# kwea123/nsff_pl

Hardware: AMD Instinct MI355X
Metric: ray-samples/sec (coarse+fine, static+dynamic) (higher is better)
Workload: dtype f16x3 (fp32 operands split into 2 halfs, 3 f16 MFMAs per product, fp32 accumulate; same 1e-4 parity as f32); 1 GPU; C2 (BASELINE.json configs[1]): static+dynamic NSFF, 1024 rays/GPU x (64 coarse + 64 importance -> 192 fine pts), train-mode fwd, fw/bw flow warp t+-1, perturb=1 noise_std=1, 8x256 MLPs, N_tau=48, all 47 outputs on device.  `value` is render_rays' throughput with autograd DISABLED (the train-mode FLAGS, inference launches: nothing kept for a backward pass); what a trainer's forward costs is aux.tra; rays_per_gpu=1024, N_samples=64, N_importance=64, parallelism=single GPU, field_launch=persistent (one workgroup per CU)

## Files before the change

### include/nsff_render.h

```cpp
#ifndef NSFF_RENDER_H
#define NSFF_RENDER_H

#include <stddef.h>
#include <stdint.h>

#ifdef __cplusplus
extern "C" {
#endif

#define NSFF_OK               0
#define NSFF_ERR_INVALID     -1
#define NSFF_ERR_NULL        -2
#define NSFF_ERR_ALIGN       -3
#define NSFF_ERR_HIP         -4

#define NSFF_ABI_VERSION      32
#define NSFF_RAW_STRIDE      16
#define NSFF_MAX_FREQS       24
#define NSFF_MAX_LAYERS       8


typedef struct NsffModelDesc {
    int32_t D;
    int32_t W;
// ... 275 lines not shown
    const float* xyz_bw;
    const float* noise_static;
    const float* noise_transient;
    const float* noise_fw;
    const float* noise_bw;
    const float* visibility;
    float* static_rgbs;  float* transient_rgbs;
    float* flows_fw;     float* flows_bw;
    float* static_sigmas; float* transient_sigmas;
    float* static_alphas; float* transient_alphas;
    float* static_weights; float* transient_weights; float* weights;
    float* xyzs_fw_bw;   float* xyzs_bw_fw;
    float* disoccs_fw;   float* disoccs_bw;
    float* depth;  float* rgb;  float* transient_alpha;  float* transient_rgb;
    float* static_only_rgb;  float* static_only_depth;
    float* xyz_exp;  float* flow_fw_exp;  float* flow_bw_exp;  float* xyz_fw_exp;  float* xyz_bw_exp;
    float* rgb_fw;   float* rgb_bw;
    float* disocc_fw;  float* disocc_bw;
    NsffFrustumArgs vis;
} NsffCompositeArgs;

int nsff_composite(const NsffCompositeArgs* args, void* stream);

int nsff_frustum_visibility(const NsffFrustumArgs* vis, const float* xyz, int64_t n_points, float* vis_count,
                            void* stream);

typedef struct NsffSplatArgs {
    int32_t H, W, n_planes;
    float   K4[4];
    float   P[12];
    float   scale;
    const float* xyz;
    const float* flow;
    const float* rgb;
    const float* alpha;
    float*       accum;
    void*        work;
    int64_t      work_bytes;
} NsffSplatArgs;
int64_t nsff_splat_work_bytes(int32_t H, int32_t W, int32_t n_planes);
int nsff_splat_planes(const NsffSplatArgs* args, void* stream);

typedef struct NsffMpiArgs {
    int32_t H, W, n_planes;
    float   dt;
    const float* accum_fw;
// ... 104 lines not shown
```

### nsff_pl_amd/_lib.py

```python
import ctypes as C
import os

import torch

_HERE = os.path.dirname(os.path.abspath(__file__))
LIB_PATH = os.environ.get("NSFF_LIB") or os.path.join(_HERE, "libnsff_hip.so")

RAW_STRIDE = 16
ABI_VERSION = 32
MAX_FREQS = 24

_ERR = {-1: "NSFF_ERR_INVALID (bad shape/flag/unsupported architecture)",
        -2: "NSFF_ERR_NULL (required pointer missing)",
        -3: "NSFF_ERR_ALIGN (pointer not 16-byte aligned)",
        -4: "NSFF_ERR_HIP"}

_fp = C.c_void_p


class ModelDesc(C.Structure):
    _fields_ = [("D", C.c_int32), ("W", C.c_int32), ("skip", C.c_int32),
                ("in_xyz", C.c_int32), ("in_dir", C.c_int32), ("in_a", C.c_int32),
                ("in_t", C.c_int32), ("use_viewdir", C.c_int32),
                ("has_transient", C.c_int32), ("has_flow", C.c_int32),
# ... 153 lines not shown
    "nsff_field_launch_plan": (C.c_int, [C.POINTER(ModelDesc), C.POINTER(FieldArgs), C.c_int32, C.c_int32, C.POINTER(C.c_int32), C.c_int32]),
    "nsff_time_bias_rows": (C.c_int, [C.POINTER(ModelDesc)]),
    "nsff_time_bias": (C.c_int, [C.POINTER(TimeBiasJob), C.c_int32, C.c_int64, C.c_void_p]),
    "nsff_rng_draws": (C.c_int, [C.POINTER(RngJob), C.c_int32, C.c_uint64, C.c_void_p]),
    "nsff_rng_draws_coarse": (C.c_int, [C.POINTER(RngJob), C.c_int32, C.c_uint64, C.POINTER(RngCoarse), C.c_void_p]),
    "nsff_side_bias": (C.c_int, [C.POINTER(ModelDesc), _fp, _fp, _fp, _fp, C.c_int64, _fp, C.c_void_p]),
    "nsff_last_hip_error": (C.c_char_p, []),
    "nsff_packed_bytes": (C.c_int, [C.POINTER(ModelDesc), C.c_int, C.POINTER(C.c_size_t)]),
    "nsff_param_count": (C.c_int, [C.POINTER(ModelDesc)]),
    "nsff_pack_weights": (C.c_int, [C.POINTER(ModelDesc), C.c_int, C.POINTER(_fp), _fp, _fp]),
    "nsff_pack_weights_ex": (C.c_int, [C.POINTER(ModelDesc), C.c_int, C.POINTER(_fp), _fp, C.c_int32, _fp]),
    "nsff_fold_heads": (C.c_int, [C.POINTER(ModelDesc), C.c_int, C.POINTER(_fp), _fp, _fp]),
    "nsff_posenc": (C.c_int, [_fp, C.c_int64, C.POINTER(C.c_float), C.c_int, _fp, _fp]),
    "nsff_time_rows": (C.c_int, [_fp, C.c_int64, C.c_int32, _fp, C.c_int64, C.c_int64, _fp, _fp, _fp]),
    "nsff_time_rows_backward": (C.c_int, [_fp, _fp, _fp, _fp, C.c_int64, C.c_int64, C.c_int64, C.c_int32, _fp, _fp]),
    "nsff_field_query": (C.c_int, [C.POINTER(ModelDesc), _fp, C.POINTER(FieldArgs), _fp]),
    "nsff_coarse_samples": (C.c_int, [_fp, C.c_int64, _fp, C.c_int32, C.c_float, _fp, _fp, _fp, _fp]),
    "nsff_fine_samples": (C.c_int, [_fp, C.c_int64, _fp, _fp, C.c_int32, C.c_int32, _fp, _fp, _fp, _fp,
                                    C.c_int32, _fp, _fp, _fp, _fp, _fp]),
    "nsff_sample_pdf": (C.c_int, [_fp, _fp, C.c_int64, C.c_int32, _fp, C.c_int32, C.c_int32,
                                  C.c_float, _fp, _fp]),
    "nsff_warp_points": (C.c_int, [_fp, _fp, _fp, C.c_int64, C.c_float, _fp, _fp, _fp]),
    "nsff_composite": (C.c_int, [C.POINTER(CompositeArgs), _fp]),
    "nsff_frustum_visibility": (C.c_int, [C.POINTER(FrustumArgs), _fp, C.c_int64, _fp, _fp]),
    "nsff_frame_rays": (C.c_int, [C.POINTER(C.c_float), C.POINTER(C.c_float), C.c_int32, C.c_int32, C.c_float,
                                  C.c_float, C.c_int64, C.c_int64, _fp, _fp]),
    "nsff_bwd_packed_bytes": (C.c_int, [C.POINTER(ModelDesc), C.POINTER(C.c_size_t)]),
    "nsff_pack_weights_bwd": (C.c_int, [C.POINTER(ModelDesc), C.POINTER(_fp), _fp, _fp]),
    "nsff_field_backward": (C.c_int, [C.POINTER(ModelDesc), _fp, C.POINTER(FieldBwdArgs), _fp]),
    "nsff_field_input_backward": (C.c_int, [_fp, C.c_int32, C.c_int32, _fp, C.c_int64, C.c_int32, C.POINTER(C.c_float), C.c_int32,
                                            C.c_int32, _fp, _fp, _fp]),
    "nsff_train_dims": (C.c_int, [C.POINTER(ModelDesc), C.POINTER(C.c_int32), C.POINTER(C.c_int32), C.POINTER(C.c_int32)]),
    "nsff_weight_grad_scratch": (C.c_int64, [C.POINTER(WgradJob), C.c_int32, C.c_int64, C.c_int32]),
    "nsff_weight_grad": (C.c_int, [C.POINTER(WgradJob), C.c_int32, C.c_int64, C.c_int32, _fp, _fp, _fp, _fp, _fp]),
    "nsff_weight_grad_accumulate": (C.c_int, [C.POINTER(WgradJob), C.c_int32, C.c_int64, C.c_int32, _fp, _fp, C.c_int64,
                                              _fp, _fp, _fp]),
    "nsff_weight_grad_accumulate_aux": (C.c_int, [C.POINTER(WgradJob), C.c_int32, C.c_int64, C.c_int32, _fp, _fp, C.c_int64,
                                                  _fp, _fp, _fp, _fp]),
    "nsff_absmax_raw": (C.c_int, [_fp, C.c_int64, _fp, _fp]),
    "nsff_last_bwd_kernel": (C.c_int, []),
    "nsff_last_bwd_grid": (C.c_int, []),
    "nsff_field_bwd_phase_program": (C.c_int, [C.POINTER(ModelDesc), C.c_int32, C.c_int32, C.c_int64, C.POINTER(C.c_uint32), C.c_int32,
                                                C.POINTER(C.c_uint32), C.c_int32]),
    "nsff_field_bwd_launch_plan": (C.c_int, [C.POINTER(ModelDesc), C.POINTER(FieldBwdArgs), C.c_int32, C.c_int32, C.c_int32,
                                             C.POINTER(C.c_int32), C.c_int32]),
    "nsff_fold_grads": (C.c_int, [C.POINTER(FoldGradArgs), _fp]),
# ... 399 lines not shown
                                  _ptr(u), samples.shape[1], int(u_per_ray), float(eps),
                                  _ptr(samples), _stream()), "nsff_sample_pdf")


def warp_points(raw, xyz, zs, z_far, xyz_fw, xyz_bw):
    _check(load().nsff_warp_points(_ptr(raw), _ptr(xyz), _ptr(zs), zs.numel(), float(z_far),
                                   _ptr(xyz_fw), _ptr(xyz_bw), _stream()), "nsff_warp_points")


def frustum_args(w2c, ts, K4, n_cams, n_frames, H, W):
    assert w2c.is_cuda and w2c.dtype == torch.float32 and w2c.is_contiguous() and w2c.shape == (n_cams * n_frames, 12)
    assert ts.is_cuda and ts.dtype == torch.int64 and ts.is_contiguous() and ts.numel() >= 1
    a = FrustumArgs(w2c=w2c.data_ptr(), ts=ts.data_ptr(), n_cams=int(n_cams), n_frames=int(n_frames), H=int(H), W=int(W))
    a.K4[:] = [float(v) for v in K4]
    a._keep = (w2c, ts)
    return a


def frustum_visibility(vis, xyz, out):
    _check(load().nsff_frustum_visibility(C.byref(vis), _ptr(xyz), xyz.shape[0], _ptr(out), _stream()),
           "nsff_frustum_visibility")


def composite(vis=None, **kw):
    a = CompositeArgs()
    for k, v in kw.items():
        if k in _COMPOSITE_PTRS_IN or k in _COMPOSITE_PTRS_OUT:
            setattr(a, k, _ptr(v))
        else:
            setattr(a, k, v)
    if vis is not None:
        a.vis = vis
    _check(load().nsff_composite(C.byref(a), _stream()), "nsff_composite")


def frame_rays(K4, c2w12, H, W, near, shift_near, first, count, rays):
    k = (C.c_float * 4)(*[float(v) for v in K4])
    m = (C.c_float * 12)(*[float(v) for v in c2w12])
    _check(load().nsff_frame_rays(k, m, int(H), int(W), float(near), float(shift_near), int(first), int(count),
                                  _ptr(rays), _stream()), "nsff_frame_rays")


BWD_PACK = 100


def bwd_packed_bytes(desc):
    n = C.c_size_t(0)
    _check(load().nsff_bwd_packed_bytes(C.byref(desc), C.byref(n)), "nsff_bwd_packed_bytes")
    return n.value


def pack_weights_bwd(desc, params, packed, fwd_packed=None):
    arr = (_fp * len(params))(*[p.data_ptr() for p in params])
    _check(load().nsff_pack_weights_bwd_ex(C.byref(desc), arr, _ptr(packed), _ptr(fwd_packed), _stream()), "nsff_pack_weights_bwd_ex")


# ... 300 lines not shown
```

### nsff_pl_amd/csrc/rays.hip

```cpp
#include <hip/hip_runtime.h>
#include <cstdlib>
#include "nsff_common.h"

namespace {

constexpr int WAVES_PER_BLOCK = 4;
constexpr int RS = NSFF_RAW_STRIDE;

__device__ __forceinline__ float wave_sum(float v) {
#pragma unroll
    for (int off = 32; off > 0; off >>= 1) v += __shfl_xor(v, off);
    return v;
}

__device__ __forceinline__ float wave_scan_mul(float v, int lane) {
#pragma unroll
    for (int off = 1; off < 64; off <<= 1) {
        const float u = __shfl_up(v, off);
        if (lane >= off) v *= u;
    }
    return v;
}
__device__ __forceinline__ float wave_scan_add(float v, int lane) {
#pragma unroll
// ... 52 lines not shown
        const int below = max(lo - 1, 0), above = min(lo, M);
        const float cb = cdf[below], ca = cdf[above];
        const float bb = bins[below], ba = bins[above];
        float denom = ca - cb;
        if (denom < eps) denom = 1.f;
        const float s = bb + (uk - cb) / denom * (ba - bb);
        if (active) {
            if (out_a) out_a[k] = s;
            if (out_b) out_b[k] = s;
        }
    }
    __syncthreads();
}

struct FineArgs {
    const float* rays; long long n_rays; const float* z_lin; const float* zs_coarse;
    int S, n_imp;
    const float* w_static; const float* w_transient;
    const float* u_static; const float* u_transient; int u_per_ray;
    float* samples_static; float* samples_transient;
    float* zs_fine; float* xyz_fine;
};

__global__ __launch_bounds__(64 * WAVES_PER_BLOCK) void fine_samples_kernel(const FineArgs a) {
    extern __shared__ __attribute__((aligned(16))) float smem[];
    const int lane = threadIdx.x & 63, wave = threadIdx.x >> 6, tid = threadIdx.x;
    constexpr int T = 64 * WAVES_PER_BLOCK;
    const long long ray = blockIdx.x;
    const int S = a.S, n_imp = a.n_imp;
    const int k_sets = a.w_transient ? 2 : 1;
    const int Sf = S + k_sets * n_imp;
    float* cdf = smem + wave * S;
    float* bins = smem + WAVES_PER_BLOCK * S;
    float* merged = bins + ((S + 3) & ~3);
    for (int j = tid; j < S - 1; j += T) bins[j] = 0.5f * (a.z_lin[j] + a.z_lin[j + 1]);
    for (int j = tid; j < S; j += T) merged[j] = a.zs_coarse[ray * S + j];
    __syncthreads();
    {
        const bool mine = wave < k_sets;
        const int set = mine ? wave : 0;
        const float* w = (set == 0 ? a.w_static : a.w_transient) + ray * S + 1;
        const float* ub = set == 0 ? a.u_static : a.u_transient;
        const float* u = a.u_per_ray ? ub + ray * n_imp : ub;
        float* keep = set == 0 ? a.samples_static : a.samples_transient;
        sample_pdf_ray(w, bins, S - 2, 1e-5f, u, n_imp, cdf, merged + S + set * n_imp,
                       keep ? keep + ray * n_imp : nullptr, lane, mine);
    }
    const float* r = a.rays + ray * 6;
    const float o0 = r[0], o1 = r[1], o2 = r[2], d0 = r[3], d1 = r[4], d2 = r[5];
    for (int i = tid; i < Sf; i += T) {
        const float v = merged[i];
        int rank = 0;
        int j = 0;
        for (; j + 4 <= Sf; j += 4) {
            const float4 o = *reinterpret_cast<const float4*>(merged + j);
            rank += (o.x < v || (o.x == v && j < i)) ? 1 : 0;
            rank += (o.y < v || (o.y == v && j + 1 < i)) ? 1 : 0;
            rank += (o.z < v || (o.z == v && j + 2 < i)) ? 1 : 0;
            rank += (o.w < v || (o.w == v && j + 3 < i)) ? 1 : 0;
        }
        for (; j < Sf; ++j) {
            const float o = merged[j];
            rank += (o < v || (o == v && j < i)) ? 1 : 0;
        }
        const long long dst = ray * Sf + rank;
        a.zs_fine[dst] = v;
        a.xyz_fine[dst * 3 + 0] = o0 + d0 * v;
        a.xyz_fine[dst * 3 + 1] = o1 + d1 * v;
        a.xyz_fine[dst * 3 + 2] = o2 + d2 * v;
    }
}

struct PdfArgs {
    const float* bins; const float* weights; long long n_rays; int M;
    const float* u; int n_imp; int u_per_ray; float eps; float* samples;
};

__global__ __launch_bounds__(64 * WAVES_PER_BLOCK) void sample_pdf_kernel(const PdfArgs a) {
    extern __shared__ __attribute__((aligned(16))) float smem[];
    const int lane = threadIdx.x & 63, wave = threadIdx.x >> 6;
    const long long ray_raw = (long long)blockIdx.x * WAVES_PER_BLOCK + wave;
    const bool active = ray_raw < a.n_rays;
    const long long ray = active ? ray_raw : a.n_rays - 1;
    float* cdf = smem + wave * (a.M + 1);
    const float* u = a.u_per_ray ? a.u + ray * a.n_imp : a.u;
    sample_pdf_ray(a.weights + ray * a.M, a.bins + ray * (a.M + 1), a.M, a.eps, u, a.n_imp, cdf,
                   active ? a.samples + ray * a.n_imp : nullptr, nullptr, lane, true);
}

struct FrameRayArgs {
    float fx, fy, cx, cy;
    float c2w[12];
    int W;
// ... 50 lines not shown
    const float ry = -rz * y * cy / fy;
    const long long frame = v.ts[0];
    float count = 0.f;
    if (frame < 0 || frame >= v.n_frames) return count;
    for (int c = 0; c < v.n_cams; ++c) {
        const float* m = v.w2c + ((long long)c * v.n_frames + frame) * 12;
        const float cam0 = fmaf(m[2], rz, fmaf(m[1], ry, m[0] * rx)) + m[3];
        const float cam1 = fmaf(m[6], rz, fmaf(m[5], ry, m[4] * rx)) + m[7];
        const float cam2 = fmaf(m[10], rz, fmaf(m[9], ry, m[8] * rx)) + m[11];
        if (!(cam2 < 0.f)) continue;
        const float c1 = -cam1, c2 = -cam2;
        const float u = fmaf(cx, c2, fx * cam0) / c2, w = fmaf(cy, c2, fy * c1) / c2;
        if (u >= 0.f && u < (float)v.W && w >= 0.f && w < (float)v.H) count += 1.f;
    }
    return count;
}

__global__ __launch_bounds__(256) void frustum_visibility_kernel(const NsffFrustumArgs v, const float* __restrict__ xyz,
                                                                 long long n_points, float* __restrict__ out) {
    const long long p = (long long)blockIdx.x * 256 + threadIdx.x;
    if (p < n_points) out[p] = frustum_count(v, xyz[3 * p], xyz[3 * p + 1], xyz[3 * p + 2]);
}

__global__ __launch_bounds__(64 * WAVES_PER_BLOCK) void composite_kernel(const NsffCompositeArgs a) {
    const int lane = threadIdx.x & 63;
    const long long ray = (long long)blockIdx.x * WAVES_PER_BLOCK + (threadIdx.x >> 6);
    if (ray >= a.n_rays) return;
    const int S = a.n_samples;
    const bool tr = a.has_transient != 0;
    const bool flows = tr && a.flow_mode >= 1;
    const bool warps = tr && a.flow_mode >= 2;

    float cT = 1.f, cTs = 1.f, cTfw = 1.f, cTbw = 1.f;
    float s_depth = 0.f, s_rgb[3] = {0, 0, 0}, s_talpha = 0.f, s_trgb[3] = {0, 0, 0};
    float s_sorgb[3] = {0, 0, 0}, s_sodepth = 0.f;
    float s_xyz[3] = {0, 0, 0}, s_ffw[3] = {0, 0, 0}, s_fbw[3] = {0, 0, 0};
    float s_rgbfw[3] = {0, 0, 0}, s_rgbbw[3] = {0, 0, 0}, s_occfw = 0.f, s_occbw = 0.f;

    for (int base = 0; base < S; base += 64) {
        const int i = base + lane;
        const bool on = i < S;
        const long long idx = ray * S + (on ? i : S - 1);
        const float z = a.zs[idx];
        const bool last = i >= S - 1;
        const float dz = last ? 0.f : a.zs[idx + 1] - z;
        const float d_s = last ? 100.f : dz;
        const float d_t = last ? 1e-3f : dz;
        const float* rec = a.raw + idx * RS;

        float sig_s = rec[3];
// ... 23 lines not shown
        cT *= __shfl(inc, 63);
        const float w = alpha * T, w_s = al_s * T, w_t = al_t * T;

        if (on) {
            if (a.static_sigmas) a.static_sigmas[idx] = sig_s;
            if (a.has_rgb && a.static_rgbs) {
                a.static_rgbs[idx * 3 + 0] = rgb_s[0]; a.static_rgbs[idx * 3 + 1] = rgb_s[1];
                a.static_rgbs[idx * 3 + 2] = rgb_s[2];
            }
            if (tr) {
                if (a.transient_sigmas) a.transient_sigmas[idx] = sig_t;
                if (a.has_rgb && a.transient_rgbs) {
                    a.transient_rgbs[idx * 3 + 0] = rgb_t[0]; a.transient_rgbs[idx * 3 + 1] = rgb_t[1];
                    a.transient_rgbs[idx * 3 + 2] = rgb_t[2];
                }
                if (a.static_alphas) a.static_alphas[idx] = al_s;
                if (a.transient_alphas) a.transient_alphas[idx] = al_t;
                if (a.static_weights) a.static_weights[idx] = w_s;
                if (a.transient_weights) a.transient_weights[idx] = w_t;
                if (a.weights) a.weights[idx] = w;
            } else {
                if (a.static_weights) a.static_weights[idx] = w;
                if (a.weights) a.weights[idx] = w;
            }
        }
        if (!a.has_rgb) continue;

        if (on) {
            s_depth += w * z;
            if (tr) {
#pragma unroll
                for (int c = 0; c < 3; ++c) { s_rgb[c] += w_s * rgb_s[c]; s_trgb[c] += w_t * rgb_t[c]; }
                s_talpha += w_t;
            } else {
#pragma unroll
                for (int c = 0; c < 3; ++c) s_rgb[c] += w * rgb_s[c];
            }
        }
        if (!tr) continue;

        {
            const float oms = on ? 1.f - al_s : 1.f;
            const float incs = wave_scan_mul(oms, lane);
            float excs = __shfl_up(incs, 1);
            if (lane == 0) excs = 1.f;
            const float Ts = cTs * excs;
// ... 89 lines not shown
        if (a.static_only_rgb) a.static_only_rgb[ray * 3 + c] = s_sorgb[c];
    }
    if (a.transient_alpha) a.transient_alpha[ray] = s_talpha;
    if (a.static_only_depth) a.static_only_depth[ray] = s_sodepth;
    if (flows) {
        for (int c = 0; c < 3; ++c) {
            if (a.xyz_exp) a.xyz_exp[ray * 3 + c] = s_xyz[c];
            if (a.flow_fw_exp) a.flow_fw_exp[ray * 3 + c] = s_ffw[c];
            if (a.flow_bw_exp) a.flow_bw_exp[ray * 3 + c] = s_fbw[c];
            if (a.xyz_fw_exp) a.xyz_fw_exp[ray * 3 + c] = s_xyz[c] + s_ffw[c];
            if (a.xyz_bw_exp) a.xyz_bw_exp[ray * 3 + c] = s_xyz[c] + s_fbw[c];
        }
    }
    if (warps) {
        for (int c = 0; c < 3; ++c) {
            if (a.rgb_fw) a.rgb_fw[ray * 3 + c] = s_rgbfw[c];
            if (a.rgb_bw) a.rgb_bw[ray * 3 + c] = s_rgbbw[c];
        }
        if (a.disocc_fw) a.disocc_fw[ray] = 1.f - fabsf(s_occfw);
        if (a.disocc_bw) a.disocc_bw[ray] = 1.f - fabsf(s_occbw);
    }
}

template <int NCH>
__global__ __launch_bounds__(64 * NCH) void composite_kernel_chunks(const NsffCompositeArgs a) {
    __shared__ float tot[NCH][4];
    __shared__ float part[NCH][32];
    const int lane = threadIdx.x & 63, c = threadIdx.x >> 6;
    const long long ray = blockIdx.x;
    const int S = a.n_samples;
    const bool tr = a.has_transient != 0;
    const bool flows = tr && a.flow_mode >= 1;
    const bool warps = tr && a.flow_mode >= 2;

    const int i = 64 * c + lane;
    const bool on = i < S;
    const long long idx = ray * S + (on ? i : S - 1);
    const float z = a.zs[idx];
    const bool last = i >= S - 1;
    const float dz = last ? 0.f : a.zs[idx + 1] - z;
    const float d_s = last ? 100.f : dz;
    const float d_t = last ? 1e-3f : dz;
    const float* rec = a.raw + idx * RS;

    float sig_s = rec[3];
    if (a.noise_static) sig_s += a.noise_static[idx] * a.noise_std;
    sig_s = softplus(sig_s);
    const float al_s = 1.f - expf(-d_s * sig_s);
    float rgb_s[3] = {0, 0, 0};
    if (a.has_rgb) { rgb_s[0] = rec[0]; rgb_s[1] = rec[1]; rgb_s[2] = rec[2]; }

    float sig_t = 0.f, al_t = 0.f, alpha = al_s;
    float rgb_t[3] = {0, 0, 0};
    if (tr) {
        sig_t = rec[7];
        if (a.visibility && a.visibility[idx] == 0.f) sig_t = -10.f;
        if (a.vis.w2c && frustum_count(a.vis, a.xyz[idx * 3], a.xyz[idx * 3 + 1], a.xyz[idx * 3 + 2]) == 0.f) sig_t = -10.f;
        if (a.noise_transient) sig_t += a.noise_transient[idx] * a.noise_std;
        sig_t = softplus(sig_t);
        al_t = 1.f - expf(-d_t * sig_t);
        alpha = 1.f - (1.f - al_s) * (1.f - al_t);
        if (a.has_rgb) { rgb_t[0] = rec[4]; rgb_t[1] = rec[5]; rgb_t[2] = rec[6]; }
    }
    const float inc = wave_scan_mul(on ? 1.f - alpha : 1.f, lane);
    float incs = 1.f, incw[2] = {1.f, 1.f}, al_tw[2] = {0.f, 0.f};
    if (a.has_rgb && tr) incs = wave_scan_mul(on ? 1.f - al_s : 1.f, lane);
    if (a.has_rgb && warps) {
#pragma unroll
        for (int dir = 0; dir < 2; ++dir) {
            const float* recw = (dir == 0 ? a.raw_fw : a.raw_bw) + idx * RS;
            const float* nz = dir == 0 ? a.noise_fw : a.noise_bw;
            float sg = recw[7];
            if (nz) sg += nz[idx] * a.noise_std;
            al_tw[dir] = 1.f - expf(-d_t * softplus(sg));
            const float al_w = 1.f - (1.f - al_s) * (1.f - al_tw[dir]);
            incw[dir] = wave_scan_mul(on ? 1.f - al_w : 1.f, lane);
        }
    }
    if (lane == 63) { tot[c][0] = inc; tot[c][1] = incs; tot[c][2] = incw[0]; tot[c][3] = incw[1]; }
    __syncthreads();
    float cT = 1.f, cTs = 1.f, cTw[2] = {1.f, 1.f};
    for (int cc = 0; cc < c; ++cc) { cT *= tot[cc][0]; cTs *= tot[cc][1]; cTw[0] *= tot[cc][2]; cTw[1] *= tot[cc][3]; }

    float exc = __shfl_up(inc, 1);
    if (lane == 0) exc = 1.f;
    const float T = cT * exc;
    const float w = alpha * T, w_s = al_s * T, w_t = al_t * T;
    if (on) {
        if (a.static_sigmas) a.static_sigmas[idx] = sig_s;
        if (a.has_rgb && a.static_rgbs) {
            a.static_rgbs[idx * 3 + 0] = rgb_s[0]; a.static_rgbs[idx * 3 + 1] = rgb_s[1];
            a.static_rgbs[idx * 3 + 2] = rgb_s[2];
        }
        if (tr) {
            if (a.transient_sigmas) a.transient_sigmas[idx] = sig_t;
// ... 25 lines not shown
#pragma unroll
            for (int k = 0; k < 3; ++k) { p[P_RGB + k] = w_s * rgb_s[k]; p[P_TRGB + k] = w_t * rgb_t[k]; }
            p[P_TALPHA] = w_t;
        } else {
#pragma unroll
            for (int k = 0; k < 3; ++k) p[P_RGB + k] = w * rgb_s[k];
        }
    }
    if (tr) {
        float excs = __shfl_up(incs, 1);
        if (lane == 0) excs = 1.f;
        const float wso = al_s * (cTs * excs);
        if (on) {
#pragma unroll
            for (int k = 0; k < 3; ++k) p[P_SORGB + k] = wso * rgb_s[k];
            p[P_SODEPTH] = wso * z;
        }
    }
    if (flows) {
        const bool far = z > a.z_far;
        float ffw[3], fbw[3], x[3];
#pragma unroll
        for (int k = 0; k < 3; ++k) {
            ffw[k] = far ? 0.f : rec[8 + k];
            fbw[k] = far ? 0.f : rec[11 + k];
            x[k] = a.xyz[idx * 3 + k];
        }
        if (on) {
#pragma unroll
            for (int k = 0; k < 3; ++k) {
                if (a.flows_fw) a.flows_fw[idx * 3 + k] = ffw[k];
                if (a.flows_bw) a.flows_bw[idx * 3 + k] = fbw[k];
                p[P_XYZ + k] = w * x[k]; p[P_FFW + k] = w * ffw[k]; p[P_FBW + k] = w * fbw[k];
            }
        }
        if (warps) {
#pragma unroll
            for (int dir = 0; dir < 2; ++dir) {
                const float* recw = (dir == 0 ? a.raw_fw : a.raw_bw) + idx * RS;
                float excw = __shfl_up(incw[dir], 1);
                if (lane == 0) excw = 1.f;
                const float Tw = cTw[dir] * excw;
                const float ws_w = al_s * Tw, wt_w = al_tw[dir] * Tw;
                if (on) {
#pragma unroll
                    for (int k = 0; k < 3; ++k) p[(dir == 0 ? P_RGBFW : P_RGBBW) + k] = ws_w * rgb_s[k] + wt_w * recw[4 + k];
                    const float* xw = (dir == 0 ? a.xyz_fw : a.xyz_bw) + idx * 3;
                    float* cyc = dir == 0 ? a.xyzs_fw_bw : a.xyzs_bw_fw;
                    const int head = dir == 0 ? 11 : 8;
                    if (cyc) {
#pragma unroll
                        for (int k = 0; k < 3; ++k) cyc[idx * 3 + k] = xw[k] + (far ? 0.f : recw[head + k]);
                    }
                    const float occ = wt_w - w_t;
                    if (dir == 0) { p[P_OCCFW] = occ; if (a.disoccs_fw) a.disoccs_fw[idx] = 1.f - fabsf(occ); }
                    else          { p[P_OCCBW] = occ; if (a.disoccs_bw) a.disoccs_bw[idx] = 1.f - fabsf(occ); }
                }
            }
        }
    }
    const int n_used = warps ? (int)P_N : (flows ? (int)P_RGBFW : (tr ? (int)P_XYZ : (int)P_TRGB));
#pragma unroll
    for (int k = 0; k < P_N; ++k) {
        if (k < n_used) {
            const float v = wave_sum(p[k]);
            if (lane == 0) part[c][k] = v;
        }
    }
    __syncthreads();
    if (threadIdx.x != 0) return;
    float s[P_N];
#pragma unroll
    for (int k = 0; k < P_N; ++k) {
        s[k] = 0.f;
        if (k < n_used) for (int cc = 0; cc < NCH; ++cc) s[k] += part[cc][k];
// ... 227 lines not shown
    if (!rays) return NSFF_ERR_NULL;
    FrameRayArgs a{};
    a.fx = K4_host[0]; a.fy = K4_host[1]; a.cx = K4_host[2]; a.cy = K4_host[3];
    for (int i = 0; i < 12; ++i) a.c2w[i] = c2w_host[i];
    a.W = W; a.near = near; a.shift_near = shift_near; a.first = first_pixel; a.count = n_pixels; a.rays = rays;
    hipLaunchKernelGGL(frame_rays_kernel, dim3((unsigned)((n_pixels + 255) / 256)), dim3(256), 0, (hipStream_t)stream, a);
    return nsff_launch_status();
}

int nsff_composite(const NsffCompositeArgs* args, void* stream) {
    if (!args) return NSFF_ERR_NULL;
    const NsffCompositeArgs& a = *args;
    if (a.n_rays < 0 || a.n_samples < 1 || a.flow_mode < 0 || a.flow_mode > 2) return NSFF_ERR_INVALID;
    if (a.n_rays == 0) return NSFF_OK;
    if (!a.raw || !a.zs) return NSFF_ERR_NULL;
    if (a.flow_mode && (!a.has_transient || !a.has_rgb)) return NSFF_ERR_INVALID;
    if (a.flow_mode >= 1 && !a.xyz) return NSFF_ERR_NULL;
    if (a.flow_mode == 2 && (!a.raw_fw || !a.raw_bw || !a.xyz_fw || !a.xyz_bw)) return NSFF_ERR_NULL;
    if (a.vis.w2c && (!a.vis.ts || !a.xyz)) return NSFF_ERR_NULL;
    if (a.vis.w2c && (a.vis.n_cams < 1 || a.vis.n_frames < 1)) return NSFF_ERR_INVALID;
    const int nch = (a.n_samples + 63) / 64;
    if (nch >= 2 && nch <= 4 && a.n_rays <= 0x7fffffffLL && getenv("NSFF_SERIAL_COMPOSITE") == nullptr) {
        const dim3 grid((unsigned)a.n_rays);
        if (nch == 2) hipLaunchKernelGGL(composite_kernel_chunks<2>, grid, dim3(128), 0, (hipStream_t)stream, a);
        else if (nch == 3) hipLaunchKernelGGL(composite_kernel_chunks<3>, grid, dim3(192), 0, (hipStream_t)stream, a);
        else hipLaunchKernelGGL(composite_kernel_chunks<4>, grid, dim3(256), 0, (hipStream_t)stream, a);
        return nsff_launch_status();
    }
    const unsigned blocks = (unsigned)((a.n_rays + WAVES_PER_BLOCK - 1) / WAVES_PER_BLOCK);
    hipLaunchKernelGGL(composite_kernel, dim3(blocks), dim3(64 * WAVES_PER_BLOCK), 0,
                       (hipStream_t)stream, a);
    return nsff_launch_status();
}

int nsff_frustum_visibility(const NsffFrustumArgs* vis, const float* xyz, int64_t n_points, float* vis_count,
                            void* stream) {
    if (!vis || !vis->w2c || !vis->ts) return NSFF_ERR_NULL;
    if (n_points < 0 || vis->n_cams < 1 || vis->n_frames < 1) return NSFF_ERR_INVALID;
    if (n_points == 0) return NSFF_OK;
    if (!xyz || !vis_count) return NSFF_ERR_NULL;
    const long long blocks = (n_points + 255) / 256;
    if (blocks > 0x7fffffffLL) return NSFF_ERR_INVALID;
    hipLaunchKernelGGL(frustum_visibility_kernel, dim3((unsigned)blocks), dim3(256), 0, (hipStream_t)stream, *vis, xyz,
                       (long long)n_points, vis_count);
    return nsff_launch_status();
}

}
```

### nsff_pl_amd/rendering.py

```python
import os

import torch

from . import _lib
from . import autograd
from . import config
from . import range_check
from . import field_grad
from . import ray_geometry

Z_FAR = 0.95

def _new(ref, *shape):
    return torch.empty(*shape, device=ref.device, dtype=torch.float32)


def sample_pdf(bins, weights, N_importance, det=False, eps=1e-5):
    _lib.require_gpu_tensor(bins, "sample_pdf bins")
    bins = bins.contiguous().float()
    weights = weights.contiguous().float()
    n_rays = weights.shape[0]
    if det:
        u = torch.linspace(0, 1, N_importance, device=bins.device)
    else:
# ... 43 lines not shown
                    add("rand", True, n_rays, N_importance)
            S = N_samples + (2 if transient else 1) * N_importance
        add("randn", noisy, n_rays, S)
        if transient:
            add("randn", noisy, n_rays, S)
            if flows and not test_time:
                add("randn", noisy, n_rays, S)
                add("randn", noisy, n_rays, S)
        self.plan = plan
        self.values = _lib.fused_draws(plan, device, need, coarse=hook)
        self.coarse_done = hook is not None

    def take(self, kind, *shape):
        if not self.fused:
            return (torch.rand if kind == "rand" else torch.randn)(*shape, device=self.device)
        if self.at >= len(self.plan) or self.plan[self.at] != (kind, shape):
            raise RuntimeError(f"draw {self.at}: {kind}{shape} is not the planned {self.plan[self.at:self.at + 1]}")
        self.at += 1
        return self.values[self.at - 1]


class _Pass:
    __slots__ = ("embeddings", "rays", "ts", "max_t", "noise_std", "test_time", "kwargs",
                 "freqs_xyz", "dir_embedded", "n_rays", "rec", "tbias", "neighbour_rows", "draws")


def _embed_rows(embeddings, key, idx):
    return embeddings[key](idx).detach().contiguous().float()


_LINSPACE = {}


def _unit_linspace(n, device):
    key = (int(n), str(device))
    if key not in _LINSPACE:
        if len(_LINSPACE) > 64:
            _LINSPACE.clear()
        _LINSPACE[key] = torch.linspace(0, 1, n, device=device)
    return _LINSPACE[key]


def _neighbour_time_rows(embeddings, ts, max_t):
    m = embeddings['t']
    if (isinstance(m, torch.nn.Embedding) and m.padding_idx is None and m.max_norm is None and m.weight.is_cuda
            and m.weight.dtype == torch.float32 and m.weight.is_contiguous() and ts.is_cuda and ts.dtype == torch.int64):
        return _lib.time_rows(m.weight.detach(), ts.contiguous(), max_t)
# ... 24 lines not shown
             and torch.is_tensor(ts) and ts.is_cuda and ts.dtype == torch.int64
             and ts.dim() == 1 and ts.shape[0] == n_rays)
    if (plan and plain and all(mod.in_channels_t == m.weight.shape[1] for _, _, mod, _ in plan)
            and not os.environ.get('NSFF_NO_TIME_INDEX')):
        outs, rows = _lib.time_bias([(mod, d) for _, _, mod, d in plan], index=(m.weight.detach(), ts.contiguous(), ctx.max_t))
        for (typ, which, _, _), out in zip(plan, outs):
            ctx.tbias[(typ, which)] = out
        if 1 in rows:
            ctx.neighbour_rows = (rows[1], rows[-1])
        return rows[0]
    t_embedded = override if override is not None else ctx.embeddings['t'](ts)
    t_embedded = t_embedded.detach().contiguous().float()
    plan = [p for p in plan if t_embedded.shape == (n_rays, p[2].in_channels_t)]
    if plan:
        if any(w == 'fw' for _, w, _, _ in plan):
            ctx.neighbour_rows = _neighbour_time_rows(ctx.embeddings, ts, ctx.max_t)
        src = {0: t_embedded, 1: ctx.neighbour_rows[0] if ctx.neighbour_rows else None, -1: ctx.neighbour_rows[1] if ctx.neighbour_rows else None}
        for (typ, which, _, _), out in zip(plan, _lib.time_bias([(mod, src[d]) for _, _, mod, d in plan])):
            ctx.tbias[(typ, which)] = out
    return t_embedded


def _inference(results, ctx, model, xyz, zs, output_transient, output_transient_flow,
               t_embedded, a_embedded):
    typ = model.typ
    n_rays, S = zs.shape
    test_time = ctx.test_time
    results[f'zs_{typ}'] = zs
    results[f'xyzs_{typ}'] = xyz
    P = n_rays * S
    sigma_only = typ == 'coarse' and test_time
    want_flow = bool(output_transient_flow) and output_transient and not sigma_only
    warps = want_flow and not test_time
    disocc = warps and 'disocc' in output_transient_flow
    if want_flow and not hasattr(model, "transient_flow_fw"):
        raise AttributeError(f"{typ} model has no flow heads")

    raw = _new(zs, P, _lib.RAW_STRIDE)
    side = dict(dir_emb=ctx.dir_embedded if model.use_viewdir and not sigma_only else None,
                a_emb=a_embedded if (model.use_viewdir and model.in_channels_a > 0 and not sigma_only) else None)
    big_enough = ctx.rec is not None or config.get_tile_points() == 130 or (config.get_tile_points() == 0 and P >= 32768)
    if (side["dir_emb"] is not None and P and S % 64 == 0 and config.get_precision() == "f16x3" and config.get_tile_points() in (0, 130)
            and big_enough and not os.environ.get('NSFF_NO_SIDE_BIAS')):
        side["s_bias"] = _lib.side_bias(model, side["dir_emb"], side["a_emb"])

    def query(tag, raw_out, pts, static_mode, transient_mode, flow_heads, t_rows, which='t', **extra):
        saves = {}
# ... 92 lines not shown
        args['transient_alphas'] = out(f'transient_alphas_{typ}', n_rays, S)

    if not sigma_only:
        args['depth'] = out(f'depth_{typ}', n_rays)
        args['rgb'] = out(f'rgb_{typ}', n_rays, 3)
        if output_transient:
            args['transient_alpha'] = out(f'transient_alpha_{typ}', n_rays)
            args['transient_rgb'] = out(f'transient_rgb_{typ}', n_rays, 3)
            args['static_only_rgb'] = out(f'_static_rgb_{typ}', n_rays, 3)
            args['static_only_depth'] = out(f'_static_depth_{typ}', n_rays)
            if want_flow:
                args['flow_mode'] = 2 if warps else 1
                args['xyz_exp'] = out('xyz_fine', n_rays, 3)
                args['flow_fw_exp'] = out('transient_flow_fw', n_rays, 3)
                args['xyz_fw_exp'] = out('xyz_fw', n_rays, 3)
                args['flow_bw_exp'] = out('transient_flow_bw', n_rays, 3)
                args['xyz_bw_exp'] = out('xyz_bw', n_rays, 3)
                if disocc:
                    args['disocc_fw'] = out('disocc_fw', n_rays, 1)
                    args['disoccs_fw'] = out('disoccs_fw', n_rays, S, 1)
                    args['disocc_bw'] = out('disocc_bw', n_rays, 1)
                    args['disoccs_bw'] = out('disoccs_bw', n_rays, S, 1)
    if n_rays:
        _lib.composite(**args)


def render_rays(models,
                embeddings,
                rays,
                ts,
                max_t,
                N_samples=64,
                perturb=0,
                noise_std=0,
                N_importance=0,
                chunk=1024 * 32,
                test_time=False,
                **kwargs):
    _lib.require_gpu_tensor(rays, "rays")
    return range_check.checked(
        "render_rays", rays.device,
        lambda: _render_rays(models, embeddings, rays, ts, max_t, N_samples, perturb, noise_std, N_importance, chunk, test_time, kwargs),
        can_fallback=bool(test_time) and perturb == 0 and noise_std == 0)


def _render_rays(models, embeddings, rays, ts, max_t, N_samples, perturb, noise_std, N_importance, chunk, test_time, kwargs,
                 fine_points=None):
    _lib.require_gpu_tensor(rays, "rays")
    _lib.load()
    want_grad = (torch.is_grad_enabled() and not test_time and
                 bool(autograd.grad_parameters(models, embeddings)))
    rec = {} if want_grad else None
    with torch.cuda.device(rays.device), torch.no_grad():
        results = {}
        rays = rays.contiguous().float()
        n_rays = rays.shape[0]
        embedding_xyz, embedding_dir = embeddings['xyz'], embeddings['dir']

        ctx = _Pass()
        ctx.embeddings, ctx.rays, ctx.ts, ctx.max_t = embeddings, rays, ts, max_t
        ctx.noise_std, ctx.test_time, ctx.kwargs, ctx.n_rays = noise_std, test_time, kwargs, n_rays
        ctx.freqs_xyz = [float(f) for f in embedding_xyz.freqs]
        ctx.rec = rec
        ctx.tbias, ctx.neighbour_rows = {}, None
        ctx.dir_embedded = None
        if any(m.use_viewdir for m in models.values()):
            view_dir = kwargs.get('view_dir', rays[:, 3:6])
            ctx.dir_embedded = embedding_dir(view_dir.contiguous().float())

        z_lin = _unit_linspace(N_samples, rays.device)
        zs = _new(rays, n_rays, N_samples)
        xyz_coarse = _new(rays, n_rays, N_samples, 3)
        ctx.draws = _Draws(rays.device, n_rays, N_samples, N_importance, perturb, noise_std, test_time, models, kwargs,
                           coarse=(rays, z_lin, zs, xyz_coarse))
        perturb_rand = ctx.draws.take("rand", n_rays, N_samples) if perturb > 0 else None
        if n_rays and not ctx.draws.coarse_done:
            _lib.coarse_samples(rays, z_lin, perturb, perturb_rand, zs, xyz_coarse)

        t_embedded = None
        if N_importance > 0:
            model = models['coarse']
            output_transient = bool(kwargs.get('output_transient', True) and model.encode_transient)
            t_embedded = _time_codes(ctx, models, kwargs, N_samples, N_importance, output_transient,
                                     kwargs.get('output_transient_flow', []))
            _inference(results, ctx, model, xyz_coarse, zs, output_transient, [], t_embedded, None)

            det = perturb == 0
            if det:
                u_s = _unit_linspace(N_importance, rays.device)
                u_t = u_s
            else:
                u_s = ctx.draws.take("rand", n_rays, N_importance)
                u_t = ctx.draws.take("rand", n_rays, N_importance) if output_transient else None
            S_fine = N_samples + (2 if output_transient else 1) * N_importance
            zs_static = _new(rays, n_rays, N_importance) if test_time else None
            zs_transient = _new(rays, n_rays, N_importance) if (test_time and output_transient) else None
            zs_fine = _new(rays, n_rays, S_fine)
            xyz_fine = _new(rays, n_rays, S_fine, 3)
            if n_rays:
                _lib.fine_samples(rays, z_lin, zs, N_importance,
                                  results['static_weights_coarse'],
                                  results['transient_weights_coarse'] if output_transient else None,
                                  u_s, u_t if output_transient else None, 0 if det else 1,
                                  zs_static, zs_transient, zs_fine, xyz_fine)
            if test_time:
                results['static_zs_fine'] = zs_static
                if output_transient:
                    results['transient_zs_fine'] = zs_transient
            if fine_points is not None:
                zs_fine, xyz_fine = fine_points(rays, zs_fine, xyz_fine)
                if tuple(zs_fine.shape) != (n_rays, S_fine) or tuple(xyz_fine.shape) != (n_rays, S_fine, 3):
                    raise ValueError(f"fine_points: expected shapes {(n_rays, S_fine)} / {(n_rays, S_fine, 3)}")
            zs, xyz = zs_fine, xyz_fine
        else:
            xyz = xyz_coarse

        model = models['fine']
        a_embedded = None
        if model.encode_appearance:
            a_embedded = kwargs['a_embedded'] if 'a_embedded' in kwargs else embeddings['a'](ts)
            a_embedded = a_embedded.detach().contiguous().float()
        if N_importance == 0:
            output_transient = bool(kwargs.get('output_transient', True) and model.encode_transient)
            t_embedded = _time_codes(ctx, models, kwargs, N_samples, 0, output_transient, kwargs.get('output_transient_flow', []))
        output_transient_flow = [] if not output_transient else kwargs.get('output_transient_flow', [])
        _inference(results, ctx, model, xyz, zs, output_transient, output_transient_flow,
                   t_embedded, a_embedded)
# ... 11 lines not shown
```

Baseline: 68.45 million ray-samples/s.

## Fuse coarse compositing with fine sample generation and stage composite records in LDS

Result: no change. 68.38 million ray-samples/s (-0.1%).

```diff
diff --git a/include/nsff_render.h b/include/nsff_render.h
--- a/include/nsff_render.h
+++ b/include/nsff_render.h
@@ -321,6 +321,12 @@
 
 int nsff_composite(const NsffCompositeArgs* args, void* stream);
 
+int nsff_coarse_stage_plan(const NsffCompositeArgs* args, int32_t n_importance);
+int nsff_composite_fine_samples(const NsffCompositeArgs* args, const float* rays, const float* z_lin, int32_t n_importance,
+                                const float* u_static, const float* u_transient, int32_t u_per_ray,
+                                float* samples_static, float* samples_transient, float* zs_fine, float* xyz_fine,
+                                void* stream);
+
 int nsff_frustum_visibility(const NsffFrustumArgs* vis, const float* xyz, int64_t n_points, float* vis_count,
                             void* stream);
 
diff --git a/nsff_pl_amd/_lib.py b/nsff_pl_amd/_lib.py
--- a/nsff_pl_amd/_lib.py
+++ b/nsff_pl_amd/_lib.py
@@ -199,6 +199,9 @@
                                   C.c_float, _fp, _fp]),
     "nsff_warp_points": (C.c_int, [_fp, _fp, _fp, C.c_int64, C.c_float, _fp, _fp, _fp]),
     "nsff_composite": (C.c_int, [C.POINTER(CompositeArgs), _fp]),
+    "nsff_coarse_stage_plan": (C.c_int, [C.POINTER(CompositeArgs), C.c_int32]),
+    "nsff_composite_fine_samples": (C.c_int, [C.POINTER(CompositeArgs), _fp, _fp, C.c_int32, _fp, _fp, C.c_int32,
+                                              _fp, _fp, _fp, _fp, _fp]),
     "nsff_frustum_visibility": (C.c_int, [C.POINTER(FrustumArgs), _fp, C.c_int64, _fp, _fp]),
     "nsff_frame_rays": (C.c_int, [C.POINTER(C.c_float), C.POINTER(C.c_float), C.c_int32, C.c_int32, C.c_float,
                                   C.c_float, C.c_int64, C.c_int64, _fp, _fp]),
@@ -644,7 +647,7 @@
            "nsff_frustum_visibility")
 
 
-def composite(vis=None, **kw):
+def _composite_args(vis, kw):
     a = CompositeArgs()
     for k, v in kw.items():
         if k in _COMPOSITE_PTRS_IN or k in _COMPOSITE_PTRS_OUT:
@@ -653,7 +656,29 @@
             setattr(a, k, v)
     if vis is not None:
         a.vis = vis
-    _check(load().nsff_composite(C.byref(a), _stream()), "nsff_composite")
+    return a
+
+
+def composite(vis=None, **kw):
+    _check(load().nsff_composite(C.byref(_composite_args(vis, kw)), _stream()), "nsff_composite")
+
+
+def coarse_stage_plan(n_importance, vis=None, **kw):
+    if os.environ.get('NSFF_NO_FUSED_COARSE'):
+        return 0
+    rc = load().nsff_coarse_stage_plan(C.byref(_composite_args(vis, kw)), int(n_importance))
+    _check(min(rc, 0), "nsff_coarse_stage_plan")
+    return rc
+
+
+def composite_fine_samples(args, rays, z_lin, n_importance, u_static, u_transient, u_per_ray, samples_static,
+                           samples_transient, zs_fine, xyz_fine):
+    vis = args.get('vis')
+    a = _composite_args(vis, {k: v for k, v in args.items() if k != 'vis'})
+    _check(load().nsff_composite_fine_samples(C.byref(a), _ptr(rays), _ptr(z_lin), int(n_importance), _ptr(u_static),
+                                              _ptr(u_transient), int(u_per_ray), _ptr(samples_static),
+                                              _ptr(samples_transient), _ptr(zs_fine), _ptr(xyz_fine), _stream()),
+           "nsff_composite_fine_samples")
 
 
 def frame_rays(K4, c2w12, H, W, near, shift_near, first, count, rays):
diff --git a/nsff_pl_amd/csrc/rays.hip b/nsff_pl_amd/csrc/rays.hip
--- a/nsff_pl_amd/csrc/rays.hip
+++ b/nsff_pl_amd/csrc/rays.hip
@@ -98,8 +98,8 @@
     float* zs_fine; float* xyz_fine;
 };
 
-__global__ __launch_bounds__(64 * WAVES_PER_BLOCK) void fine_samples_kernel(const FineArgs a) {
-    extern __shared__ __attribute__((aligned(16))) float smem[];
+__device__ __forceinline__ void fine_samples_ray(const FineArgs& a, float* smem, const float* w_static_row,
+                                                 const float* w_transient_row) {
     const int lane = threadIdx.x & 63, wave = threadIdx.x >> 6, tid = threadIdx.x;
     constexpr int T = 64 * WAVES_PER_BLOCK;
     const long long ray = blockIdx.x;
@@ -115,7 +115,7 @@
     {
         const bool mine = wave < k_sets;
         const int set = mine ? wave : 0;
-        const float* w = (set == 0 ? a.w_static : a.w_transient) + ray * S + 1;
+        const float* w = (set == 0 ? w_static_row : w_transient_row) + 1;
         const float* ub = set == 0 ? a.u_static : a.u_transient;
         const float* u = a.u_per_ray ? ub + ray * n_imp : ub;
         float* keep = set == 0 ? a.samples_static : a.samples_transient;
@@ -145,6 +145,12 @@
         a.xyz_fine[dst * 3 + 1] = o1 + d1 * v;
         a.xyz_fine[dst * 3 + 2] = o2 + d2 * v;
     }
+}
+
+__global__ __launch_bounds__(64 * WAVES_PER_BLOCK) void fine_samples_kernel(const FineArgs a) {
+    extern __shared__ __attribute__((aligned(16))) float smem[];
+    const long long ray = blockIdx.x;
+    fine_samples_ray(a, smem, a.w_static + ray * a.S, a.w_transient ? a.w_transient + ray * a.S : nullptr);
 }
 
 struct PdfArgs {
@@ -241,10 +247,8 @@
     if (p < n_points) out[p] = frustum_count(v, xyz[3 * p], xyz[3 * p + 1], xyz[3 * p + 2]);
 }
 
-__global__ __launch_bounds__(64 * WAVES_PER_BLOCK) void composite_kernel(const NsffCompositeArgs a) {
-    const int lane = threadIdx.x & 63;
-    const long long ray = (long long)blockIdx.x * WAVES_PER_BLOCK + (threadIdx.x >> 6);
-    if (ray >= a.n_rays) return;
+__device__ __forceinline__ void composite_ray(const NsffCompositeArgs& a, const long long ray, const int lane,
+                                              float* keep_ws, float* keep_wt) {
     const int S = a.n_samples;
     const bool tr = a.has_transient != 0;
     const bool flows = tr && a.flow_mode >= 1;
@@ -314,6 +318,10 @@
             } else {
                 if (a.static_weights) a.static_weights[idx] = w;
                 if (a.weights) a.weights[idx] = w;
+            }
+            if (keep_ws) {
+                keep_ws[i] = tr ? w_s : w;
+                if (tr) keep_wt[i] = w_t;
             }
         }
         if (!a.has_rgb) continue;
@@ -449,8 +457,27 @@
     }
 }
 
-template <int NCH>
+__global__ __launch_bounds__(64 * WAVES_PER_BLOCK) void composite_kernel(const NsffCompositeArgs a) {
+    const long long ray = (long long)blockIdx.x * WAVES_PER_BLOCK + (threadIdx.x >> 6);
+    if (ray >= a.n_rays) return;
+    composite_ray(a, ray, threadIdx.x & 63, nullptr, nullptr);
+}
+
+__global__ __launch_bounds__(64 * WAVES_PER_BLOCK) void coarse_composite_fine_kernel(const NsffCompositeArgs c, const FineArgs f) {
+    extern __shared__ __attribute__((aligned(16))) float smem[];
+    const long long ray = blockIdx.x;
+    const int S = f.S;
+    const int Sf = S + (f.w_transient ? 2 : 1) * f.n_imp;
+    float* rows = smem + WAVES_PER_BLOCK * S + ((S + 3) & ~3) + ((Sf + 3) & ~3);
+    if ((threadIdx.x >> 6) == 0) composite_ray(c, ray, threadIdx.x & 63, rows, rows + S);
+    fine_samples_ray(f, smem, rows, f.w_transient ? rows + S : nullptr);
+}
+
+constexpr int REC_LDS = 64 * (RS + 1);
+
+template <int NCH, bool STAGE>
 __global__ __launch_bounds__(64 * NCH) void composite_kernel_chunks(const NsffCompositeArgs a) {
+    extern __shared__ __attribute__((aligned(16))) float smem[];
     __shared__ float tot[NCH][4];
     __shared__ float part[NCH][32];
     const int lane = threadIdx.x & 63, c = threadIdx.x >> 6;
@@ -469,25 +496,51 @@
     const float d_s = last ? 100.f : dz;
     const float d_t = last ? 1e-3f : dz;
     const float* rec = a.raw + idx * RS;
-
-    float sig_s = rec[3];
+    const int n_sets = warps ? 3 : 1;
+    const int li = (on ? lane : S - 1 - 64 * c) * (RS + 1);
+    const float* srec = smem + c * n_sets * REC_LDS;
+    if (STAGE) {
+        const int nv = min(64, S - 64 * c);
+        const long long first = (ray * S + 64 * c) * RS;
+#pragma unroll
+        for (int set = 0; set < 3; ++set) {
+            if (set < n_sets) {
+                const float4* g = reinterpret_cast<const float4*>((set == 0 ? a.raw : (set == 1 ? a.raw_fw : a.raw_bw)) + first);
+                float* dst = smem + (c * n_sets + set) * REC_LDS;
+#pragma unroll
+                for (int j = 0; j < 4; ++j) {
+                    const int q = lane + 64 * j, r = q >> 2;
+                    if (r < nv) {
+                        const float4 v = g[q];
+                        float* d = dst + r * (RS + 1) + 4 * (q & 3);
+                        d[0] = v.x; d[1] = v.y; d[2] = v.z; d[3] = v.w;
+                    }
+                }
+            }
+        }
+        __syncthreads();
+    }
+    auto R = [&](int k) -> float { return STAGE ? srec[li + k] : rec[k]; };
+    auto RW = [&](int dir, const float* recw, int k) -> float { return STAGE ? srec[(1 + dir) * REC_LDS + li + k] : recw[k]; };
+
+    float sig_s = R(3);
     if (a.noise_static) sig_s += a.noise_static[idx] * a.noise_std;
     sig_s = softplus(sig_s);
     const float al_s = 1.f - expf(-d_s * sig_s);
     float rgb_s[3] = {0, 0, 0};
-    if (a.has_rgb) { rgb_s[0] = rec[0]; rgb_s[1] = rec[1]; rgb_s[2] = rec[2]; }
+    if (a.has_rgb) { rgb_s[0] = R(0); rgb_s[1] = R(1); rgb_s[2] = R(2); }
 
     float sig_t = 0.f, al_t = 0.f, alpha = al_s;
     float rgb_t[3] = {0, 0, 0};
     if (tr) {
-        sig_t = rec[7];
+        sig_t = R(7);
         if (a.visibility && a.visibility[idx] == 0.f) sig_t = -10.f;
         if (a.vis.w2c && frustum_count(a.vis, a.xyz[idx * 3], a.xyz[idx * 3 + 1], a.xyz[idx * 3 + 2]) == 0.f) sig_t = -10.f;
         if (a.noise_transient) sig_t += a.noise_transient[idx] * a.noise_std;
         sig_t = softplus(sig_t);
         al_t = 1.f - expf(-d_t * sig_t);
         alpha = 1.f - (1.f - al_s) * (1.f - al_t);
-        if (a.has_rgb) { rgb_t[0] = rec[4]; rgb_t[1] = rec[5]; rgb_t[2] = rec[6]; }
+        if (a.has_rgb) { rgb_t[0] = R(4); rgb_t[1] = R(5); rgb_t[2] = R(6); }
     }
     const float inc = wave_scan_mul(on ? 1.f - alpha : 1.f, lane);
     float incs = 1.f, incw[2] = {1.f, 1.f}, al_tw[2] = {0.f, 0.f};
@@ -497,7 +550,7 @@
         for (int dir = 0; dir < 2; ++dir) {
             const float* recw = (dir == 0 ? a.raw_fw : a.raw_bw) + idx * RS;
             const float* nz = dir == 0 ? a.noise_fw : a.noise_bw;
-            float sg = recw[7];
+            float sg = RW(dir, recw, 7);
             if (nz) sg += nz[idx] * a.noise_std;
             al_tw[dir] = 1.f - expf(-d_t * softplus(sg));
             const float al_w = 1.f - (1.f - al_s) * (1.f - al_tw[dir]);
@@ -569,8 +622,8 @@
         float ffw[3], fbw[3], x[3];
 #pragma unroll
         for (int k = 0; k < 3; ++k) {
-            ffw[k] = far ? 0.f : rec[8 + k];
-            fbw[k] = far ? 0.f : rec[11 + k];
+            ffw[k] = far ? 0.f : R(8 + k);
+            fbw[k] = far ? 0.f : R(11 + k);
             x[k] = a.xyz[idx * 3 + k];
         }
         if (on) {
@@ -591,13 +644,13 @@
                 const float ws_w = al_s * Tw, wt_w = al_tw[dir] * Tw;
                 if (on) {
 #pragma unroll
-                    for (int k = 0; k < 3; ++k) p[(dir == 0 ? P_RGBFW : P_RGBBW) + k] = ws_w * rgb_s[k] + wt_w * recw[4 + k];
+                    for (int k = 0; k < 3; ++k) p[(dir == 0 ? P_RGBFW : P_RGBBW) + k] = ws_w * rgb_s[k] + wt_w * RW(dir, recw, 4 + k);
                     const float* xw = (dir == 0 ? a.xyz_fw : a.xyz_bw) + idx * 3;
                     float* cyc = dir == 0 ? a.xyzs_fw_bw : a.xyzs_bw_fw;
                     const int head = dir == 0 ? 11 : 8;
                     if (cyc) {
 #pragma unroll
-                        for (int k = 0; k < 3; ++k) cyc[idx * 3 + k] = xw[k] + (far ? 0.f : recw[head + k]);
+                        for (int k = 0; k < 3; ++k) cyc[idx * 3 + k] = xw[k] + (far ? 0.f : RW(dir, recw, head + k));
                     }
                     const float occ = wt_w - w_t;
                     if (dir == 0) { p[P_OCCFW] = occ; if (a.disoccs_fw) a.disoccs_fw[idx] = 1.f - fabsf(occ); }
@@ -871,14 +924,57 @@
     const int nch = (a.n_samples + 63) / 64;
     if (nch >= 2 && nch <= 4 && a.n_rays <= 0x7fffffffLL && getenv("NSFF_SERIAL_COMPOSITE") == nullptr) {
         const dim3 grid((unsigned)a.n_rays);
-        if (nch == 2) hipLaunchKernelGGL(composite_kernel_chunks<2>, grid, dim3(128), 0, (hipStream_t)stream, a);
-        else if (nch == 3) hipLaunchKernelGGL(composite_kernel_chunks<3>, grid, dim3(192), 0, (hipStream_t)stream, a);
-        else hipLaunchKernelGGL(composite_kernel_chunks<4>, grid, dim3(256), 0, (hipStream_t)stream, a);
+        const bool warps = a.has_transient && a.flow_mode >= 2;
+        const uintptr_t addr = (uintptr_t)a.raw | (warps ? (uintptr_t)a.raw_fw | (uintptr_t)a.raw_bw : 0);
+        if (!(addr & 15) && getenv("NSFF_NO_STAGED_COMPOSITE") == nullptr) {
+            const size_t lds = (size_t)nch * (warps ? 3 : 1) * REC_LDS * sizeof(float);
+            if (nch == 2) hipLaunchKernelGGL((composite_kernel_chunks<2, true>), grid, dim3(128), lds, (hipStream_t)stream, a);
+            else if (nch == 3) hipLaunchKernelGGL((composite_kernel_chunks<3, true>), grid, dim3(192), lds, (hipStream_t)stream, a);
+            else hipLaunchKernelGGL((composite_kernel_chunks<4, true>), grid, dim3(256), lds, (hipStream_t)stream, a);
+            return nsff_launch_status();
+        }
+        if (nch == 2) hipLaunchKernelGGL((composite_kernel_chunks<2, false>), grid, dim3(128), 0, (hipStream_t)stream, a);
+        else if (nch == 3) hipLaunchKernelGGL((composite_kernel_chunks<3, false>), grid, dim3(192), 0, (hipStream_t)stream, a);
+        else hipLaunchKernelGGL((composite_kernel_chunks<4, false>), grid, dim3(256), 0, (hipStream_t)stream, a);
         return nsff_launch_status();
     }
     const unsigned blocks = (unsigned)((a.n_rays + WAVES_PER_BLOCK - 1) / WAVES_PER_BLOCK);
     hipLaunchKernelGGL(composite_kernel, dim3(blocks), dim3(64 * WAVES_PER_BLOCK), 0,
                        (hipStream_t)stream, a);
+    return nsff_launch_status();
+}
+
+int nsff_coarse_stage_plan(const NsffCompositeArgs* args, int32_t n_importance) {
+    if (!args) return NSFF_ERR_NULL;
+    const NsffCompositeArgs& a = *args;
+    if (a.n_rays < 0 || a.n_samples < 1 || n_importance < 0) return NSFF_ERR_INVALID;
+    if (n_importance < 1 || a.n_rays < 1 || a.n_rays > 0x7fffffffLL) return 0;
+    if (a.n_samples != 64 || !a.has_rgb || a.flow_mode != 0 || a.visibility || a.vis.w2c) return 0;
+    if (!a.static_weights || (a.has_transient && !a.transient_weights)) return 0;
+    const int Sf = a.n_samples + (a.has_transient ? 2 : 1) * n_importance;
+    const size_t lds = (size_t)(WAVES_PER_BLOCK * a.n_samples + ((a.n_samples + 3) & ~3) + ((Sf + 3) & ~3) + 2 * a.n_samples) * sizeof(float);
+    return lds <= 64 * 1024 ? 1 : 0;
+}
+
+int nsff_composite_fine_samples(const NsffCompositeArgs* args, const float* rays, const float* z_lin, int32_t n_importance,
+                                const float* u_static, const float* u_transient, int32_t u_per_ray,
+                                float* samples_static, float* samples_transient, float* zs_fine, float* xyz_fine,
+                                void* stream) {
+    const int plan = nsff_coarse_stage_plan(args, n_importance);
+    if (plan < 0) return plan;
+    if (args->n_rays == 0) return NSFF_OK;
+    if (plan != 1) return NSFF_ERR_INVALID;
+    const NsffCompositeArgs& a = *args;
+    if (!a.raw || !a.zs || !rays || !z_lin || !u_static || !zs_fine || !xyz_fine) return NSFF_ERR_NULL;
+    if (a.has_transient && !u_transient) return NSFF_ERR_NULL;
+    const int S = a.n_samples;
+    FineArgs f{rays, (long long)a.n_rays, z_lin, a.zs, S, n_importance,
+               a.static_weights, a.has_transient ? a.transient_weights : nullptr, u_static, u_transient, u_per_ray,
+               samples_static, samples_transient, zs_fine, xyz_fine};
+    const int Sf = S + (a.has_transient ? 2 : 1) * n_importance;
+    const size_t lds = (size_t)(WAVES_PER_BLOCK * S + ((S + 3) & ~3) + ((Sf + 3) & ~3) + 2 * S) * sizeof(float);
+    hipLaunchKernelGGL(coarse_composite_fine_kernel, dim3((unsigned)a.n_rays), dim3(64 * WAVES_PER_BLOCK), lds,
+                       (hipStream_t)stream, a, f);
     return nsff_launch_status();
 }
 
diff --git a/nsff_pl_amd/rendering.py b/nsff_pl_amd/rendering.py
--- a/nsff_pl_amd/rendering.py
+++ b/nsff_pl_amd/rendering.py
@@ -89,7 +89,7 @@
 
 class _Pass:
     __slots__ = ("embeddings", "rays", "ts", "max_t", "noise_std", "test_time", "kwargs",
-                 "freqs_xyz", "dir_embedded", "n_rays", "rec", "tbias", "neighbour_rows", "draws")
+                 "freqs_xyz", "dir_embedded", "n_rays", "rec", "tbias", "neighbour_rows", "draws", "n_importance")
 
 
 def _embed_rows(embeddings, key, idx):
@@ -160,7 +160,7 @@
 
 
 def _inference(results, ctx, model, xyz, zs, output_transient, output_transient_flow,
-               t_embedded, a_embedded):
+               t_embedded, a_embedded, fine_stage=None):
     typ = model.typ
     n_rays, S = zs.shape
     test_time = ctx.test_time
@@ -299,7 +299,11 @@
                     args['disocc_bw'] = out('disocc_bw', n_rays, 1)
                     args['disoccs_bw'] = out('disoccs_bw', n_rays, S, 1)
     if n_rays:
+        if fine_stage is not None and _lib.coarse_stage_plan(ctx.n_importance, **args) == 1:
+            _lib.composite_fine_samples(args, **fine_stage())
+            return True
         _lib.composite(**args)
+    return False
 
 
 def render_rays(models,
@@ -339,6 +343,7 @@
         ctx.noise_std, ctx.test_time, ctx.kwargs, ctx.n_rays = noise_std, test_time, kwargs, n_rays
         ctx.freqs_xyz = [float(f) for f in embedding_xyz.freqs]
         ctx.rec = rec
+        ctx.n_importance = N_importance
         ctx.tbias, ctx.neighbour_rows = {}, None
         ctx.dir_embedded = None
         if any(m.use_viewdir for m in models.values()):
@@ -360,26 +365,32 @@
             output_transient = bool(kwargs.get('output_transient', True) and model.encode_transient)
             t_embedded = _time_codes(ctx, models, kwargs, N_samples, N_importance, output_transient,
                                      kwargs.get('output_transient_flow', []))
-            _inference(results, ctx, model, xyz_coarse, zs, output_transient, [], t_embedded, None)
-
             det = perturb == 0
-            if det:
-                u_s = _unit_linspace(N_importance, rays.device)
-                u_t = u_s
-            else:
-                u_s = ctx.draws.take("rand", n_rays, N_importance)
-                u_t = ctx.draws.take("rand", n_rays, N_importance) if output_transient else None
             S_fine = N_samples + (2 if output_transient else 1) * N_importance
             zs_static = _new(rays, n_rays, N_importance) if test_time else None
             zs_transient = _new(rays, n_rays, N_importance) if (test_time and output_transient) else None
             zs_fine = _new(rays, n_rays, S_fine)
             xyz_fine = _new(rays, n_rays, S_fine, 3)
-            if n_rays:
-                _lib.fine_samples(rays, z_lin, zs, N_importance,
-                                  results['static_weights_coarse'],
-                                  results['transient_weights_coarse'] if output_transient else None,
-                                  u_s, u_t if output_transient else None, 0 if det else 1,
-                                  zs_static, zs_transient, zs_fine, xyz_fine)
+
+            def fine_stage():
+                if det:
+                    u_s = _unit_linspace(N_importance, rays.device)
+                    u_t = u_s
+                else:
+                    u_s = ctx.draws.take("rand", n_rays, N_importance)
+                    u_t = ctx.draws.take("rand", n_rays, N_importance) if output_transient else None
+                return dict(rays=rays, z_lin=z_lin, n_importance=N_importance, u_static=u_s,
+                            u_transient=u_t if output_transient else None, u_per_ray=0 if det else 1,
+                            samples_static=zs_static, samples_transient=zs_transient, zs_fine=zs_fine, xyz_fine=xyz_fine)
+
+            if not _inference(results, ctx, model, xyz_coarse, zs, output_transient, [], t_embedded, None, fine_stage=fine_stage):
+                f = fine_stage()
+                if n_rays:
+                    _lib.fine_samples(rays, z_lin, zs, N_importance,
+                                      results['static_weights_coarse'],
+                                      results['transient_weights_coarse'] if output_transient else None,
+                                      f['u_static'], f['u_transient'], f['u_per_ray'],
+                                      zs_static, zs_transient, zs_fine, xyz_fine)
             if test_time:
                 results['static_zs_fine'] = zs_static
                 if output_transient:
```
